# tskare/gpuaudiobench

Hardware: AMD Instinct MI355X
Metric: audio_buffers_per_sec (higher is better)
Workload: dtype f32

## Files before the change

### gpuaudiobench_amd/csrc/k_conv_accel.hip

```cpp
#include <hip/hip_runtime.h>
#include <hip/hip_ext.h>

#include <cmath>
#include <cstdlib>
#include <algorithm>
#include <chrono>
#include <memory>
#include <mutex>
#include <string>
#include <thread>
#include <type_traits>
#include <utility>
#include <vector>

#include "gab_common.hpp"
#include "gab_fft.hpp"
#include "gab_plan.hpp"
#include "k_conv_fdl.hpp"

namespace gab {
namespace fft {

void build_twiddles(float* t) {
    for (int m = 0; m < kTwiddleN; ++m) {
// ... 404 lines not shown
    load_spectra<kNB, 16>(cb, pmF + (size_t)q * kBinsB, tid);
    typename FB::Twiddles twb;
    FB::expand_twiddles(twb_base, twb);
    FB::run(zb, X, Y, twb, tid);
    cf zpb[16];
    partner_exchange<kNB, 16, true>(zb, zpb, X, tid);
    spectral_product<kNB, 16>(zb, zpb, cb, tid);
    FBi::template run<typename FB::Twiddles, 4>(zb, Y, X, twb, tid);
    cf* const c1 = cp + ((head + 1) & (kCarrySlots - 1)) * kB;
    cf* const c2 = cp + ((head + 2) & (kCarrySlots - 1)) * kB;
    c1[tid] = zb[12];
    c1[tid + kThreads] = zb[13];
    c2[tid] = zb[14];
    c2[tid + kThreads] = zb[15];
}

constexpr unsigned kRtSentinel = 0xffa5c3e1u;
__device__ __forceinline__ bool rt_pending(unsigned w) { return (w >> 24) == (kRtSentinel >> 24); }
constexpr size_t kRtUploadPiece = (size_t(4) << 20) - 256;
constexpr int kRtPollLimit = 1 << 21;
constexpr int kRtMaxGroups = 40;
constexpr size_t kBatchChunk = 256;
struct ConvRoundTrip {
    unsigned* stage;
    float* park;
    float* h_out;
    unsigned* counters;
    unsigned* done;
    const unsigned* landed;
    unsigned* error;
    unsigned epoch;
    int groups;
    unsigned bound[kRtMaxGroups + 1];
};

#ifdef GAB_ABLATE
__device__ unsigned long long g_rt_stamps[65 * 4];
#define GAB_RT_STAMP_MIN(g, i) do { if (threadIdx.x == 0) atomicMin(&g_rt_stamps[(g) * 4 + (i)], (unsigned long long)__builtin_amdgcn_s_memrealtime()); } while (0)
#define GAB_RT_STAMP_MAX(g, i) do { if (threadIdx.x == 0) atomicMax(&g_rt_stamps[(g) * 4 + (i)], (unsigned long long)__builtin_amdgcn_s_memrealtime()); } while (0)
#else
#define GAB_RT_STAMP_MIN(g, i) do {} while (0)
#define GAB_RT_STAMP_MAX(g, i) do {} while (0)
#endif

__device__ __forceinline__ unsigned rt_peek(const unsigned* p) {
    return __hip_atomic_load(p, __ATOMIC_RELAXED, __HIP_MEMORY_SCOPE_SYSTEM);
}
constexpr unsigned kRtErrWait = 1u, kRtErrTorn = 2u;

__global__ __launch_bounds__(kThreads) void conv_round_trip_check_kernel(unsigned* __restrict__ stage, const float* __restrict__ hist,
                                                                        unsigned* __restrict__ verdict, int slot) {
    const int tid = threadIdx.x, q = blockIdx.x;
    const cf* const hp = reinterpret_cast<const cf*>(hist) + ((size_t)q * kSlots + slot) * kB;
    unsigned* const row = stage + (size_t)(2 * q) * kB;
    const cf c0 = hp[tid], c1 = hp[tid + kThreads];
    const unsigned v0 = rt_peek(row + tid), v1 = rt_peek(row + tid + kThreads), v2 = rt_peek(row + kB + tid), v3 = rt_peek(row + kB + tid + kThreads);
    const bool torn = v0 != __float_as_uint(c0.x) || v2 != __float_as_uint(c0.y) || v1 != __float_as_uint(c1.x) || v3 != __float_as_uint(c1.y);
    if (torn) __hip_atomic_fetch_or(verdict, kRtErrTorn, __ATOMIC_RELAXED, __HIP_MEMORY_SCOPE_SYSTEM);
    __hip_atomic_store(row + tid, kRtSentinel, __ATOMIC_RELAXED, __HIP_MEMORY_SCOPE_SYSTEM);
    __hip_atomic_store(row + tid + kThreads, kRtSentinel, __ATOMIC_RELAXED, __HIP_MEMORY_SCOPE_SYSTEM);
    __hip_atomic_store(row + kB + tid, kRtSentinel, __ATOMIC_RELAXED, __HIP_MEMORY_SCOPE_SYSTEM);
    __hip_atomic_store(row + kB + tid + kThreads, kRtSentinel, __ATOMIC_RELAXED, __HIP_MEMORY_SCOPE_SYSTEM);
}

__global__ __launch_bounds__(kThreads, 2) void conv_round_trip_kernel(
    ConvRoundTrip rt, float* __restrict__ hist, const float4* __restrict__ pmA, const float4* __restrict__ pmB,
    const cf* __restrict__ tw, int T, int head) {
    __shared__ cf lds[2 * kLdsHalf];
    __shared__ int s_word;
    cf* const lds0 = lds;
    cf* const lds1 = lds + kLdsHalf;
    const int tid = threadIdx.x;
    const int q = blockIdx.x;
    const int ta = 2 * q;
    int g = 0;
    while (q >= (int)rt.bound[g + 1]) ++g;
    GAB_RT_STAMP_MIN(g, 0);
    cf* const hp = reinterpret_cast<cf*>(hist) + (size_t)q * kSlots * kB;
    using FA = fft::BlockFFT<kNA, 4, false>;
    using FAi = fft::BlockFFT<kNA, 4, true>;
    using FB = fft::BlockFFT<kNB, 16, false>;
    using FBi = fft::BlockFFT<kNB, 16, true>;

    cf zb[16];
    typename FB::Bases twb_base;
    FB::load_twiddles(twb_base, tw, tid);
#pragma unroll
    for (int r = 0; r < 16; ++r) zb[r] = hp[((head + (r >> 1)) & (kSlots - 1)) * kB + (r & 1) * kThreads + tid];
    const cf prev0 = zb[14], prev1 = zb[15];
    {
        float4 cb[16];
        load_spectra<kNB, 16>(cb, pmB + (size_t)q * kBinsB, tid);
        __builtin_amdgcn_sched_barrier(0);
        typename FB::Twiddles twb;
        FB::expand_twiddles(twb_base, twb);
        FB::run(zb, lds1, lds0, twb, tid);
        cf zpb[16];
        partner_exchange<kNB, 16, true>(zb, zpb, lds1, tid);
        spectral_product<kNB, 16>(zb, zpb, cb, tid);
        FBi::template run<typename FB::Twiddles, 2>(zb, lds0, lds1, twb, tid);
    }
    const cf far0 = zb[14], far1 = zb[15];

    float4 ca[4];
    load_spectra<kNA, 4>(ca, pmA + (size_t)q * kBinsA, tid);
    typename FA::Twiddles twa;
    {
        typename FA::Bases twa_base;
        FA::load_twiddles(twa_base, tw, tid);
        FA::expand_twiddles(twa_base, twa);
    }

    const unsigned* const row = rt.stage + (size_t)ta * kB;
    if (tid == 0) {
        int tries = 0, bad = 0;
        while (rt_pending(rt_peek(row + 2 * kB - 1))) {
            if ((++tries & 63) == 0 && rt_peek(rt.landed) == rt.epoch) break;
            if (tries > kRtPollLimit) { bad = 1; break; }
            __builtin_amdgcn_s_sleep(30);
        }
        s_word = bad;
    }
    __syncthreads();
    bool gave_up = s_word != 0;
    unsigned w[4];
    {
        int tries = 0;
        for (;;) {
            w[0] = rt_peek(row + tid);
            w[1] = rt_peek(row + tid + kThreads);
            w[2] = rt_peek(row + kB + tid);
            w[3] = rt_peek(row + kB + tid + kThreads);
            if (gave_up || !(rt_pending(w[0]) || rt_pending(w[1]) || rt_pending(w[2]) || rt_pending(w[3]))) break;
            if ((++tries & 15) == 0 && __hip_atomic_load(rt.landed, __ATOMIC_ACQUIRE, __HIP_MEMORY_SCOPE_SYSTEM) == rt.epoch) {
                w[0] = rt_peek(row + tid);
                w[1] = rt_peek(row + tid + kThreads);
                w[2] = rt_peek(row + kB + tid);
                w[3] = rt_peek(row + kB + tid + kThreads);
                break;
            }
            if (tries > kRtPollLimit) { gave_up = true; break; }
            __builtin_amdgcn_s_sleep(10);
        }
    }
    GAB_RT_STAMP_MAX(g, 1);
    if (gave_up) __hip_atomic_store(rt.error, kRtErrWait, __ATOMIC_RELAXED, __HIP_MEMORY_SCOPE_SYSTEM);

    cf za[4];
    za[0] = prev0;
    za[1] = prev1;
    za[2] = mk(__uint_as_float(w[0]), __uint_as_float(w[2]));
    za[3] = mk(__uint_as_float(w[1]), __uint_as_float(w[3]));
    hp[head * kB + tid] = za[2];
    hp[head * kB + kThreads + tid] = za[3];
    __syncthreads();
    FA::run(za, lds0, lds1, twa, tid);
    {
        cf zpa[4];
        partner_exchange<kNA, 4, true>(za, zpa, lds0, tid);
        spectral_product<kNA, 4>(za, zpa, ca, tid);
    }
    FAi::run(za, lds1, lds0, twa, tid);
    float ya0 = 0.f, yb0 = 0.f, ya1 = 0.f, yb1 = 0.f;
    ya0 += za[2].x; yb0 += za[2].y; ya1 += za[3].x; yb1 += za[3].y;
    ya0 += far0.x; yb0 += far0.y; ya1 += far1.x; yb1 += far1.y;

    {
        unsigned long long* const p0 = reinterpret_cast<unsigned long long*>(rt.park + (size_t)T * tid + ta);
        unsigned long long* const p1 = reinterpret_cast<unsigned long long*>(rt.park + (size_t)T * (tid + kThreads) + ta);
        const unsigned long long v0 = ((unsigned long long)__float_as_uint(yb0) << 32) | __float_as_uint(ya0);
        const unsigned long long v1 = ((unsigned long long)__float_as_uint(yb1) << 32) | __float_as_uint(ya1);
        __hip_atomic_store(p0, v0, __ATOMIC_RELAXED, __HIP_MEMORY_SCOPE_AGENT);
        __hip_atomic_store(p1, v1, __ATOMIC_RELAXED, __HIP_MEMORY_SCOPE_AGENT);
    }
    asm volatile("s_waitcnt vmcnt(0)" ::: "memory");
    __syncthreads();
    GAB_RT_STAMP_MAX(g, 2);
    const int first = rt.bound[g];
    const int members = (int)rt.bound[g + 1] - first;
    unsigned* const gw = rt.counters + 32 * g;
    if (tid == 0) {
        const unsigned old = __hip_atomic_fetch_add(&gw[0], 1u, __ATOMIC_RELAXED, __HIP_MEMORY_SCOPE_AGENT);
        int role = 1;
        if (old + 1u == rt.epoch * (unsigned)members) {
            role = 2;
            __hip_atomic_store(&gw[1], 0u, __ATOMIC_RELAXED, __HIP_MEMORY_SCOPE_AGENT);
            asm volatile("s_waitcnt vmcnt(0)" ::: "memory");
            __hip_atomic_store(&gw[2], rt.epoch, __ATOMIC_RELAXED, __HIP_MEMORY_SCOPE_AGENT);
        } else {
            int tries = 0;
            while (__hip_atomic_load(&gw[2], __ATOMIC_RELAXED, __HIP_MEMORY_SCOPE_AGENT) != rt.epoch) {
                if (++tries > (1 << 10)) { role = 0; break; }
                __builtin_amdgcn_s_sleep(3);
            }
        }
        s_word = role;
    }
    __syncthreads();
    const int role = s_word;
    if (role == 0) return;
    const int row_f4 = members / 2;
    const auto srd = __builtin_amdgcn_make_buffer_rsrc(rt.park, 0, (int)((size_t)T * kB * 4), 0x00020000);
    const int col0 = 2 * first;
    unsigned drained = 0;
    for (;;) {
        __syncthreads();
        if (tid == 0) s_word = (int)__hip_atomic_fetch_add(&gw[1], 1u, __ATOMIC_RELAXED, __HIP_MEMORY_SCOPE_AGENT);
        __syncthreads();
        const int share = s_word;
        if (share >= members) break;
        const int i = share * kThreads + tid;
        const int sidx = i / row_f4, c = i - sidx * row_f4;
        const auto raw = __builtin_amdgcn_raw_buffer_load_b128(srd, 4u * (unsigned)(T * sidx + col0 + 4 * c), 0, 16);
        typedef float f4v __attribute__((ext_vector_type(4)));
        const f4v val = {__uint_as_float(raw[0]), __uint_as_float(raw[1]), __uint_as_float(raw[2]), __uint_as_float(raw[3])};
        float* const dst = rt.h_out + (size_t)T * sidx + col0 + 4 * c;
        asm volatile("global_store_dwordx4 %0, %1, off sc0 sc1" ::"v"(dst), "v"(val) : "memory");
        ++drained;
        if (role != 2) break;
    }
    asm volatile("s_waitcnt vmcnt(0)" ::: "memory");
    __syncthreads();
    GAB_RT_STAMP_MAX(g, 3);
    if (tid == 0 && drained) {
        const unsigned old = __hip_atomic_fetch_add(&rt.counters[32 * rt.groups], drained, __ATOMIC_RELAXED, __HIP_MEMORY_SCOPE_AGENT);
        if (old + drained == rt.epoch * (unsigned)gridDim.x) {
            __hip_atomic_store(rt.done, rt.epoch, __ATOMIC_RELAXED, __HIP_MEMORY_SCOPE_SYSTEM);
            GAB_RT_STAMP_MAX(64, 0);
        }
    }
}

__global__ __launch_bounds__(kThreads, 2) void conv_batch_kernel(
    const float* __restrict__ in, float* __restrict__ out, float* __restrict__ hist,
    const float4* __restrict__ pmA, const float4* __restrict__ pmB,
    const cf* __restrict__ tw, int T, int head, int n_buffers) {
    __shared__ cf lds[2 * kLdsHalf];
    const size_t step = (size_t)T * kB;
    for (int nb = 0; nb < n_buffers; ++nb)
        conv_one_buffer<true, true, true>(in + nb * step, out + nb * step, hist, pmA, pmB, tw, T,
                                             (head + nb) & (kSlots - 1), lds);
}

constexpr int kBatchBarriers = 6;

struct ConvEngine {
    const unsigned* doorbell;
    unsigned* relay;
    unsigned* progress;
    unsigned* completed;
    unsigned* error;
    int ring;
    int poll_every_period;
    unsigned* started;
    unsigned* resident;
    unsigned long long idle_ticks;
};
constexpr double kEngineIdleSeconds = 4.0;

typedef unsigned u4 __attribute__((ext_vector_type(4)));

constexpr int kB12Threads = 768;
constexpr int kB12SpecCf = 4 * kBinsA * 2;
constexpr int kB12Tw1Cf = 16 * 15;
constexpr int kB12Lds = 6 * kWaveImg + 2 * kLdsHalf + kB12SpecCf + kB12Tw1Cf;

template <int N, int R, int R0, int R1, class PM>
__device__ __forceinline__ void load_spectra_part(float4 (&c)[R1 - R0], PM pm, int tid) {
    constexpr int NT = N / R;
#pragma unroll
    for (int r = R0; r < R1; ++r) {
        const int k = tid + r * NT;
        if (r < R / 2) c[r - R0] = pm[k];
        else if (r > R / 2) c[r - R0] = pm[N - k];
        else c[r - R0] = pm[tid == 0 ? k : N - k];
    }
}
template <int N, int R, int R0, int R1>
__device__ __forceinline__ void spectral_product_part(cf (&z)[R], const cf (&zraw)[R1 - R0], const float4 (&c)[R1 - R0], int tid) {
#pragma unroll
    for (int r = R0; r < R1; ++r) {
        cf P = mk(c[r - R0].x, c[r - R0].y), M = mk(c[r - R0].z, c[r - R0].w);
        if (r > R / 2 || (r == R / 2 && tid != 0)) z[r] = fft::cfma_cjcj(zraw[r - R0], M, fft::cmulc(z[r], P));
        else z[r] = fft::cfma_cj(zraw[r - R0], M, fft::cmul(z[r], P));
    }
}
template <int N, int R, int R0, int R1>
__device__ __forceinline__ void spectral_product_partner_part(cf (&wp)[R1 - R0], const cf (&z)[R], const cf (&zp)[R1 - R0], const float4 (&c)[R1 - R0]) {
    static_assert(R1 <= R / 2, "the partners of the low bins");
#pragma unroll
    for (int r = R0; r < R1; ++r) {
        cf P = mk(c[r - R0].x, c[r - R0].y), M = mk(c[r - R0].z, c[r - R0].w);
        wp[r - R0] = fft::cfma_cjcj(z[r], M, fft::cmulc(zp[r - R0], P));
    }
}
template <int R0, int R1>
__device__ __forceinline__ void near_product_half(cf (&v)[16], const cf* fimg, const float4* sp_lds, int lane) {
    cf zp[R1 - R0];
    float4 ch[R1 - R0];
#pragma unroll
    for (int r = R0; r < R1; ++r) zp[r - R0] = fimg[PadA16::at((kNA - (lane + 64 * r)) & (kNA - 1))];
    load_spectra_part<kNA, 16, R0, R1>(ch, sp_lds, lane);
    spectral_product_part<kNA, 16, R0, R1>(v, zp, ch, lane);
}

#ifdef GAB_ABLATE
__device__ unsigned long long g_split_stamps[2 * 8 * 8192];
#define GAB_B12BAR(period, i)                                                                                         \
    do {                                                                                                              \
        if ((sp.debug & 64) && ((period) == 32 || (period) == 33) && lane == 0)                                       \
            g_split_stamps[(((size_t)blockIdx.x * 12 + w) * 2 + ((period) - 32)) * 6 + (i)] = __builtin_amdgcn_s_memrealtime(); \
        __syncthreads();                                                                                              \
    } while (0)
#else
#define GAB_B12BAR(period, i) __syncthreads()
#endif
__device__ __forceinline__ void conv_split_batch12_resident(
    const float* __restrict__ in, float* __restrict__ out, float* __restrict__ hist,
    const float4* __restrict__ pmA, const ConvSplit& sp, const cf* __restrict__ tw, int T, int head0, int n_buffers,
    cf* __restrict__ lds) {
    cf* const far_img = lds + 6 * kWaveImg;
    float4* const spec = reinterpret_cast<float4*>(far_img + 2 * kLdsHalf);
    cf* const tw1 = reinterpret_cast<cf*>(spec + 4 * kBinsA);
    const int tid = threadIdx.x;
    const int d = xcd_contiguous(blockIdx.x, gridDim.x);
    const size_t step = (size_t)T * kB;
    {
        const float4* const gA = pmA + (size_t)(2 * d) * kBinsA;
        const float4* const gA2 = sp.pmA2 + (size_t)(2 * d) * kBinsA;
        for (int i = tid; i < 2 * kBinsA; i += kB12Threads) { spec[i] = gA[i]; spec[2 * kBinsA + i] = gA2[i]; }
        if (tid < 16) {
            cf pw[15];
            fft::powers_of<16>(tw[tid * (fft::kTwiddleN / 256)], pw);
#pragma unroll
            for (int r = 0; r < 15; ++r) tw1[tid * 15 + r] = pw[r];
        }
    }
    __syncthreads();
    const int lane = tid & 63;
    const int w = __builtin_amdgcn_readfirstlane(tid >> 6);
    const unsigned rb = (unsigned)lane + ((unsigned)lane >> 4);
    auto in_slot = [&](int slot) -> const float* { return in + (size_t)slot * step; };
    auto idle_period = [&]() { for (int i = 0; i < kBatchBarriers; ++i) __syncthreads(); };

    if (w >= 4) {
        const int g = __builtin_amdgcn_readfirstlane((w - 4) >> 2);
        const int ft = (tid - kThreads) & (kThreads - 1);
        cf* const img = far_img + g * kLdsHalf;
        const int q = 2 * d + g;
        const cf* const hp = reinterpret_cast<const cf*>(hist) + (size_t)q * kSlots * kB;
        cf* const cg = sp.carry + (size_t)q * kCarrySlots * kB;
        const size_t ca = (size_t)(2 * q) * kB, cb_ = ca + kB;
        const float4* const pf = sp.pmF + (size_t)q * kBinsB;
        using B16 = fft::Butterfly<16, false>;
        using B16i = fft::Butterfly<16, true>;
        cf tw2[15];
        fft::powers_of<16>(tw[ft], tw2);
        auto opaque_t = [&]() -> unsigned { unsigned v = (unsigned)ft; asm volatile("" : "+v"(v)); return v; };
        auto w0_of = [](unsigned t) -> unsigned { return t * 17u; };
        auto rd_of = [](unsigned t) -> unsigned { return t + (t >> 4); };
        auto w1_of = [](unsigned t) -> unsigned { const unsigned b1 = (t >> 4) * 256u + (t & 15u); return b1 + (b1 >> 4); };
        auto tw1row_of = [&](unsigned t) -> const cf* { return tw1 + (t & 15u) * 15u; };
        auto load_window = [&](auto part_tag, int nb, cf (&z)[16]) {
            constexpr int PART = decltype(part_tag)::value;
            const int head = (head0 + nb) & (kSlots - 1);
            int fo = ft;
            asm volatile("" : "+v"(fo));
            if constexpr (PART == 0) {
                const float* const cur = in_slot(nb);
                z[14] = mk(cur[ca + fo], cur[cb_ + fo]);
                z[15] = mk(cur[ca + fo + kThreads], cur[cb_ + fo + kThreads]);
            }
            constexpr int BL0 = PART == 0 ? 4 : 0, BL1 = PART == 0 ? 7 : 4;
            if (nb >= kSlots - 1) {
#pragma unroll
                for (int bl = BL0; bl < BL1; ++bl) {
                    const float* const src = in_slot(nb - (7 - bl));
                    z[2 * bl] = mk(src[ca + fo], src[cb_ + fo]);
                    z[2 * bl + 1] = mk(src[ca + fo + kThreads], src[cb_ + fo + kThreads]);
                }
            } else {
#pragma unroll
                for (int bl = BL0; bl < BL1; ++bl) {
                    if (nb - 7 + bl >= 0) {
                        const float* const src = in_slot(nb - (7 - bl));
                        z[2 * bl] = mk(src[ca + fo], src[cb_ + fo]);
                        z[2 * bl + 1] = mk(src[ca + fo + kThreads], src[cb_ + fo + kThreads]);
                    } else {
                        const int s = ((head + 1 + bl) & (kSlots - 1)) * kB;
                        z[2 * bl] = hp[s + fo];
                        z[2 * bl + 1] = hp[s + kThreads + fo];
                    }
                }
            }
        };
        cf z[16], zn[16];
#ifdef GAB_ABLATE
        const bool own_bins = (sp.debug & 128) != 0;
#else
        constexpr bool own_bins = false;
#endif
        auto first_half = [&](int nb) {
#pragma unroll
            for (int r = 0; r < 16; ++r) z[r] = zn[r];
            B16::run(z);
            {
                const unsigned w0 = w0_of(opaque_t());
#pragma unroll
                for (int r = 0; r < 16; ++r) img[w0 + r] = z[B16::out_slot(r)];
            }
            GAB_B12BAR(nb, 0);
            {
                const unsigned t = opaque_t(), rd = rd_of(t);
                const cf* const tw1row = tw1row_of(t);
#pragma unroll
                for (int r = 0; r < 16; ++r) z[r] = img[rd + 272 * r];
#pragma unroll
                for (int r = 1; r < 16; ++r) z[r] = fft::cmul(z[r], tw1row[r - 1]);
            }
            B16::run(z);
            GAB_B12BAR(nb, 1);
            {
                const unsigned w1 = w1_of(opaque_t());
#pragma unroll
                for (int r = 0; r < 16; ++r) img[w1 + 17 * r] = z[B16::out_slot(r)];
            }
            __builtin_amdgcn_sched_barrier(0);
            float4 clo[8], cny = make_float4(0.0f, 0.0f, 0.0f, 0.0f);
            {
                int fo = ft;
                asm volatile("" : "+v"(fo));
                load_spectra_part<kNB, 16, 0, 8>(clo, pf, fo);
                if (fo == 0) cny = pf[kNB / 2];
            }
            __builtin_amdgcn_sched_barrier(0);
            GAB_B12BAR(nb, 2);
            {
                const unsigned rd = rd_of(opaque_t());
#pragma unroll
                for (int r = 0; r < 16; ++r) z[r] = img[rd + 272 * r];
            }
#pragma unroll
            for (int r = 1; r < 16; ++r) z[r] = fft::cmul(z[r], tw2[r - 1]);
            B16::run(z);
            GAB_B12BAR(nb, 3);
#ifdef GAB_ABLATE
            if (own_bins) {
                {
                    const unsigned t = opaque_t();
#pragma unroll
                    for (int r = 0; r < 16; ++r) img[t + 256u * r] = z[B16::out_slot(r)];
                }
                GAB_B12BAR(nb, 4);
                cf o[16];
#pragma unroll
                for (int r = 0; r < 16; ++r) o[r] = z[B16::out_slot(r)];
#pragma unroll
                for (int r = 0; r < 16; ++r) z[r] = o[r];
                const unsigned t = opaque_t();
                const cf* const pb = img + (kNB - 256 * 15) - t;
                cf zp[8];
                zp[0] = img[(kNB - t) & (kNB - 1)];
#pragma unroll
                for (int r = 1; r < 8; ++r) zp[r] = pb[256 * (15 - r)];
                spectral_product_part<kNB, 16, 0, 8>(z, zp, clo, ft);
                load_spectra_part<kNB, 16, 8, 16>(clo, pf, ft);
#pragma unroll
                for (int r = 0; r < 8; ++r) zp[r] = pb[256 * (7 - r)];
                spectral_product_part<kNB, 16, 8, 16>(z, zp, clo, ft);
                GAB_B12BAR(nb, 5);
                return;
            }
#endif
            {
                const unsigned t = opaque_t();
#pragma unroll
                for (int r = 8; r < 16; ++r) img[t + 256u * (r - 8)] = z[B16::out_slot(r)];
            }
            GAB_B12BAR(nb, 4);
            {
                cf o[16];
#pragma unroll
                for (int r = 0; r < 16; ++r) o[r] = z[B16::out_slot(r)];
#pragma unroll
                for (int r = 0; r < 16; ++r) z[r] = o[r];
                const unsigned t = opaque_t();
                const cf* const pb = img + (kNB / 2 - 256 * 7) - t;
                cf zp[8], wp[8];
                zp[0] = img[(kNB / 2 - t) & (kNB / 2 - 1)];
                if (t == 0) zp[0] = z[0];
#pragma unroll
                for (int r = 1; r < 8; ++r) zp[r] = pb[256 * (7 - r)];
                spectral_product_partner_part<kNB, 16, 0, 8>(wp, z, zp, clo);
                spectral_product_part<kNB, 16, 0, 8>(z, zp, clo, ft);
                if (t == 0) {
                    const cf P = mk(cny.x, cny.y), M = mk(cny.z, cny.w);
                    wp[0] = fft::cfma_cj(z[8], M, fft::cmul(z[8], P));
                }
                cf* const qb = img + kNB / 2 + (kNB / 2 - 256 * 7) - t;
                img[kNB / 2 + ((kNB / 2 - t) & (kNB / 2 - 1))] = wp[0];
#pragma unroll
                for (int r = 1; r < 8; ++r) qb[256 * (7 - r)] = wp[r];
            }
            GAB_B12BAR(nb, 5);
        };
        auto second_half = [&](int period, int nb_done, int nb_next) {
            if (nb_next >= 0) {
                load_window(std::integral_constant<int, 0>{}, nb_next, zn);
            } else {
#pragma unroll
                for (int r = 0; r < 16; ++r) zn[r] = mk(0.0f, 0.0f);
            }
            __builtin_amdgcn_sched_barrier(0);
            if (nb_done >= 0) {
                if (!own_bins) {
                    const unsigned t = opaque_t();
#pragma unroll
                    for (int r = 8; r < 16; ++r) z[r] = img[kNB / 2 + t + 256u * (r - 8)];
                }
                B16i::run(z);
            }
            GAB_B12BAR(period, 0);
            if (nb_done >= 0) {
                const unsigned w0 = w0_of(opaque_t());
#pragma unroll
                for (int r = 0; r < 16; ++r) img[w0 + r] = z[B16i::out_slot(r)];
            }
            GAB_B12BAR(period, 1);
            if (nb_done >= 0) {
                const unsigned t = opaque_t(), rd = rd_of(t);
                const cf* const tw1row = tw1row_of(t);
#pragma unroll
                for (int r = 0; r < 16; ++r) z[r] = img[rd + 272 * r];
#pragma unroll
                for (int r = 1; r < 16; ++r) z[r] = fft::cmulc(z[r], tw1row[r - 1]);
                B16i::run(z);
            }
            GAB_B12BAR(period, 2);
            if (nb_done >= 0) {
                const unsigned w1 = w1_of(opaque_t());
#pragma unroll
                for (int r = 0; r < 16; ++r) img[w1 + 17 * r] = z[B16i::out_slot(r)];
            }
            __builtin_amdgcn_sched_barrier(0);
            if (nb_next >= 0) load_window(std::integral_constant<int, 1>{}, nb_next, zn);
            __builtin_amdgcn_sched_barrier(0);
            GAB_B12BAR(period, 3);
            if (nb_done >= 0) {
                const unsigned rd = rd_of(opaque_t());
#pragma unroll
                for (int r = 0; r < 16; ++r) z[r] = img[rd + 272 * r];
#pragma unroll
                for (int r = 1; r < 16; ++r) z[r] = fft::cmulc(z[r], tw2[r - 1]);
                cf x12, x13, x14, x15;
                B16i::run_last4(z, x12, x13, x14, x15);
                const int head = (head0 + nb_done) & (kSlots - 1);
                cf* const c1 = cg + ((head + 1) & (kCarrySlots - 1)) * kB;
                cf* const c2 = cg + ((head + 2) & (kCarrySlots - 1)) * kB;
                c1[ft] = x12;
                c1[ft + kThreads] = x13;
                c2[ft] = x14;
                c2[ft + kThreads] = x15;
            }
            GAB_B12BAR(period, 4);
            if (nb_done >= 0) asm volatile("s_waitcnt vmcnt(0)" ::: "memory");
            GAB_B12BAR(period, 5);
        };
        const int first = (g - head0) & 1;
        int nb = 0;
        if (first == 0 && n_buffers > 0) {
            load_window(std::integral_constant<int, 0>{}, 0, zn);
            load_window(std::integral_constant<int, 1>{}, 0, zn);
        }
        __syncthreads();
        if (first == 1) {
            second_half(0, -1, 1 < n_buffers ? 1 : -1);
            nb = 1;
        }
        for (;;) {
            if (nb > n_buffers) break;
            if (nb < n_buffers) first_half(nb); else idle_period();
            ++nb;
            if (nb > n_buffers) break;
            second_half(nb, nb - 1 < n_buffers ? nb - 1 : -1, nb + 1 < n_buffers ? nb + 1 : -1);
            ++nb;
        }
    } else if (w < 2) {
        const int q = 2 * d + w;
        cf* const hp = reinterpret_cast<cf*>(hist) + (size_t)q * kSlots * kB;
        cf* const img = lds + w * kWaveImg;
        cf* const hand = lds + (2 + w) * kWaveImg;
        const float4* const sa = spec + w * kBinsA;
        const float4* const sa2 = spec + (2 + w) * kBinsA;
        using WF = fft::WaveFFT1024<false>;
        WF::Lean t;
        WF::load_twiddles(t, tw, lane);
        const size_t xoff = (size_t)(2 * q) * kB;
        cf z[16], prev[8], nxt[8];
        {
            const int s1 = ((head0 + kSlots - 1) & (kSlots - 1)) * kB, s2 = ((head0 + kSlots - 2) & (kSlots - 1)) * kB;
#pragma unroll
            for (int j = 0; j < 8; ++j) z[j] = hp[s2 + lane + 64 * j];
#pragma unroll
            for (int j = 0; j < 8; ++j) prev[j] = hp[s1 + lane + 64 * j];
            if (n_buffers > 0) {
                const float* const x0 = in_slot(0) + xoff;
#pragma unroll
                for (int j = 0; j < 8; ++j) nxt[j] = mk(x0[lane + 64 * j], x0[kB + lane + 64 * j]);
            }
#pragma unroll
            for (int j = 0; j < 8; ++j) z[8 + j] = prev[j];
            WF::run(z, img, t, lane, WF::NoHook());
#pragma unroll
            for (int r = 0; r < 16; ++r) img[rb + 68 * r] = z[r];
            __syncthreads();
        }
        for (int nb = 0; nb < n_buffers; ++nb) {
            const int head = (head0 + nb) & (kSlots - 1);
            cf share[16];
#pragma unroll
            for (int r = 0; r < 8; ++r) share[r] = img[rb + 68 * r];
            near_product_half<0, 8>(share, img, sa2, lane);
            GAB_B12BAR(nb, 0);
            __builtin_amdgcn_sched_barrier(0);
#pragma unroll
            for (int j = 0; j < 8; ++j) { z[j] = prev[j]; z[8 + j] = nxt[j]; }
            if (nb + kSlots >= n_buffers) {
#pragma unroll
                for (int j = 0; j < 8; ++j) hp[head * kB + lane + 64 * j] = nxt[j];
            }
#pragma unroll
            for (int j = 0; j < 8; ++j) prev[j] = nxt[j];
            if (nb + 1 < n_buffers) {
                int lo = lane;
                asm volatile("" : "+v"(lo));
                const float* const xa = in_slot(nb + 1) + xoff + lo;
#pragma unroll
                for (int j = 0; j < 8; ++j) nxt[j] = mk(xa[64 * j], xa[kB + 64 * j]);
            }
            WF::run(z, img, t, lane, [&](int i) { GAB_B12BAR(nb, 1 + i); });
#pragma unroll
            for (int r = 0; r < 16; ++r) img[rb + 68 * r] = z[r];
            GAB_B12BAR(nb, 3);
            near_product_half<0, 8>(z, img, sa, lane);
            GAB_B12BAR(nb, 4);
#pragma unroll
            for (int r = 0; r < 8; ++r) hand[rb + 68 * r] = fft::cadd(z[r], share[r]);
            GAB_B12BAR(nb, 5);
        }
        idle_period();
    } else {
        const int pr = w - 2;
        cf* const hand = lds + (2 + pr) * kWaveImg;
        const cf* const fimg = lds + pr * kWaveImg;
        const float4* const sa = spec + pr * kBinsA;
        const float4* const sa2 = spec + (2 + pr) * kBinsA;
        cf* const img = lds + (4 + pr) * kWaveImg;
        const cf* const other = lds + (4 + (1 - pr)) * kWaveImg;
        const cf* const cg = sp.carry + (size_t)(2 * d + pr) * kCarrySlots * kB;
        using WFi = fft::WaveFFT1024<true>;
        WFi::Lean t;
        WFi::load_twiddles(t, tw, lane);
        cf ws[16], sum[8];
        auto product_half = [&](const float4* sp_lds) {
#pragma unroll
            for (int r = 8; r < 16; ++r) ws[r] = fimg[rb + 68 * r];
            near_product_half<8, 16>(ws, fimg, sp_lds, lane);
        };
        auto store_share = [&]() {
#pragma unroll
            for (int r = 8; r < 16; ++r) hand[rb + 68 * r] = ws[r];
        };
        auto sum_halves = [&]() {
#pragma unroll
            for (int j = 0; j < 8; ++j) sum[j] = fft::cadd(ws[8 + j], hand[rb + 68 * (8 + j)]);
        };
        __syncthreads();
        if (n_buffers > 0) {
            product_half(sa2);
            GAB_B12BAR(0, 0);
            store_share();
            GAB_B12BAR(0, 1);
            GAB_B12BAR(0, 2);
            GAB_B12BAR(0, 3);
            product_half(sa);
            GAB_B12BAR(0, 4);
            sum_halves();
            GAB_B12BAR(0, 5);
        } else {
            idle_period();
        }
        for (int nb = 1; nb <= n_buffers; ++nb) {
            const bool products = nb < n_buffers;
            const int b = nb - 1;
            const int head = (head0 + b) & (kSlots - 1);
            float* const outb = out + (size_t)b * step;
            cf z[16], y[8], park[8];
#pragma unroll
            for (int r = 0; r < 8; ++r) z[r] = hand[rb + 68 * r];
#pragma unroll
            for (int j = 0; j < 8; ++j) z[8 + j] = sum[j];
            {
                int lo = lane;
                asm volatile("" : "+v"(lo));
                const unsigned long long* const cy = reinterpret_cast<const unsigned long long*>(cg + (head & (kCarrySlots - 1)) * kB + lo);
#pragma unroll
                for (int j = 0; j < 8; ++j) {
                    const unsigned long long v = __hip_atomic_load(cy + 64 * j, __ATOMIC_RELAXED, __HIP_MEMORY_SCOPE_AGENT);
                    park[j] = mk(__uint_as_float((unsigned)v), __uint_as_float((unsigned)(v >> 32)));
                }
            }
            __builtin_amdgcn_sched_barrier(0);
            if (products) product_half(sa2);
            GAB_B12BAR(nb, 0);
            if (products) store_share();
            __builtin_amdgcn_sched_barrier(0);
            WFi::run(z, img, t, lane, [&](int i) { GAB_B12BAR(nb, 1 + i); });
#pragma unroll
            for (int j = 0; j < 8; ++j) y[j] = fft::cadd(z[8 + j], park[j]);
            GAB_B12BAR(nb, 3);
            if (pr == 0) {
#pragma unroll
                for (int j = 0; j < 4; ++j) img[lane + 64 * j] = y[4 + j];
            } else {
#pragma unroll
                for (int j = 0; j < 4; ++j) img[lane + 64 * j] = y[j];
            }
            __builtin_amdgcn_sched_barrier(0);
            if (products) product_half(sa);
            GAB_B12BAR(nb, 4);
            {
                float* const o0 = outb + 4 * (size_t)d;
                if (pr == 0) {
#pragma unroll
                    for (int j = 0; j < 4; ++j) {
                        const cf theirs = other[lane + 64 * j];
                        *reinterpret_cast<float4*>(o0 + (size_t)T * (lane + 64 * j)) = make_float4(y[j].x, y[j].y, theirs.x, theirs.y);
                    }
                } else {
#pragma unroll
                    for (int j = 0; j < 4; ++j) {
                        const cf theirs = other[lane + 64 * j];
                        *reinterpret_cast<float4*>(o0 + (size_t)T * (lane + 64 * (4 + j))) = make_float4(theirs.x, theirs.y, y[4 + j].x, y[4 + j].y);
                    }
                }
            }
            if (products) sum_halves();
            GAB_B12BAR(nb, 5);
        }
    }
}

__global__ __launch_bounds__(kB12Threads) void conv_split_batch12_kernel(
    const float* __restrict__ in, float* __restrict__ out, float* __restrict__ hist,
    const float4* __restrict__ pmA, ConvSplit sp, const cf* __restrict__ tw, int T, int head0, int n_buffers) {
    __shared__ __attribute__((aligned(16))) cf lds[kB12Lds];
    conv_split_batch12_resident(in, out, hist, pmA, sp, tw, T, head0, n_buffers, lds);
}

#ifdef GAB_ABLATE
#define GAB_E12BAR(i)                                                                                                 \
    do {                                                                                                              \
        if ((sp.debug & 64) && (nb == 4000 || nb == 4001) && lane == 0)                                               \
            g_split_stamps[(((size_t)blockIdx.x * 12 + w) * 2 + (nb - 4000)) * 6 + (i)] = __builtin_amdgcn_s_memrealtime(); \
        __syncthreads();                                                                                              \
    } while (0)
#else
#define GAB_E12BAR(i) __syncthreads()
#endif
__device__ __forceinline__ void conv_split_engine12_resident(
    const float* __restrict__ in, float* __restrict__ out, float* __restrict__ hist,
    const float4* __restrict__ pmA, const ConvSplit& sp, const cf* __restrict__ tw, int T, int head0,
    const ConvEngine& eng, cf* __restrict__ lds, unsigned* __restrict__ s_door) {
    constexpr bool ENGINE = true;
    constexpr int n_buffers = 0;
    (void)ENGINE; (void)n_buffers;
    cf* const far_img = lds + 6 * kWaveImg;
    float4* const spec = reinterpret_cast<float4*>(far_img + 2 * kLdsHalf);
    cf* const tw1 = reinterpret_cast<cf*>(spec + 4 * kBinsA);
    const int tid = threadIdx.x;
    const int d = xcd_contiguous(blockIdx.x, gridDim.x);
    const size_t step = (size_t)T * kB;
    {
        const float4* const gA = pmA + (size_t)(2 * d) * kBinsA;
        const float4* const gA2 = sp.pmA2 + (size_t)(2 * d) * kBinsA;
        for (int i = tid; i < 2 * kBinsA; i += kB12Threads) { spec[i] = gA[i]; spec[2 * kBinsA + i] = gA2[i]; }
        if (tid < 16) {
            cf pw[15];
            fft::powers_of<16>(tw[tid * (fft::kTwiddleN / 256)], pw);
#pragma unroll
            for (int r = 0; r < 15; ++r) tw1[tid * 15 + r] = pw[r];
        }
    }
    constexpr int kPoller = 2 * 64;
    auto read_door = [&]() -> unsigned {
        if (blockIdx.x == 0) {
            const unsigned v = __hip_atomic_load(eng.doorbell, __ATOMIC_RELAXED, __HIP_MEMORY_SCOPE_SYSTEM);
            __hip_atomic_store(eng.relay, v, __ATOMIC_RELAXED, __HIP_MEMORY_SCOPE_AGENT);
            return v;
        }
        return __hip_atomic_load(eng.relay, __ATOMIC_RELAXED, __HIP_MEMORY_SCOPE_AGENT);
    };
    if (tid == 0) {
        s_door[2] = 0;
        const unsigned before = __hip_atomic_fetch_add(eng.started, 1u, __ATOMIC_RELAXED, __HIP_MEMORY_SCOPE_AGENT);
        if (before == 0) __hip_atomic_store(&eng.resident[0], 1u, __ATOMIC_RELAXED, __HIP_MEMORY_SCOPE_SYSTEM);
        if (before + 1 == gridDim.x) __hip_atomic_store(&eng.resident[1], gridDim.x, __ATOMIC_RELAXED, __HIP_MEMORY_SCOPE_SYSTEM);
    }
    __syncthreads();
    const int lane = tid & 63;
    const int w = __builtin_amdgcn_readfirstlane(tid >> 6);
    const unsigned rb = (unsigned)lane + ((unsigned)lane >> 4);
    const bool aggregator = blockIdx.x == (gridDim.x > 1 ? 1u : 0u);
    unsigned reported = 0;
    auto aggregate_request = [&](u4& a, u4& b) {
        const auto srd = __builtin_amdgcn_make_buffer_rsrc(eng.progress, 0, (int)(8u * gridDim.x), 0x00020000);
        a = __builtin_amdgcn_raw_buffer_load_b128(srd, 32u * (unsigned)lane, 0, 16);
        b = __builtin_amdgcn_raw_buffer_load_b128(srd, 32u * (unsigned)lane + 16u, 0, 16);
    };
    auto aggregate_report = [&](const u4& a, const u4& b) {
        const unsigned words = 2u * gridDim.x;
        auto pick = [&](unsigned v, unsigned idx) { return idx < words ? v : 0xffffffffu; };
        unsigned m = min(min(min(pick(a[0], 8u * lane), pick(a[1], 8u * lane + 1)), min(pick(a[2], 8u * lane + 2), pick(a[3], 8u * lane + 3))),
                         min(min(pick(b[0], 8u * lane + 4), pick(b[1], 8u * lane + 5)), min(pick(b[2], 8u * lane + 6), pick(b[3], 8u * lane + 7))));
// ... 1823 lines not shown
```

Baseline: 213,300.

## Pair mirror bins in-register via lane-half swaps instead of LDS round trip

Remaps which frequency bins each far-path thread owns so that a bin and its conjugate partner live in the two halves of the same wavefront. The partner values are then exchanged with cross-lane half swaps rather than being written to and read back from LDS. This removes LDS stores and loads in the spectral product stage and the second-half reload. In exchange it adds cross-lane permute traffic and special-case selects for lanes 0 and 32 of the first wave, and it changes the thread-to-bin mapping that other stages rely on.

```diff
diff --git a/gpuaudiobench_amd/csrc/k_conv_accel.hip b/gpuaudiobench_amd/csrc/k_conv_accel.hip
--- a/gpuaudiobench_amd/csrc/k_conv_accel.hip
+++ b/gpuaudiobench_amd/csrc/k_conv_accel.hip
@@ -730,6 +730,12 @@
     for (int r = R0; r < R1; ++r) zp[r - R0] = fimg[PadA16::at((kNA - (lane + 64 * r)) & (kNA - 1))];
     load_spectra_part<kNA, 16, R0, R1>(ch, sp_lds, lane);
     spectral_product_part<kNA, 16, R0, R1>(v, zp, ch, lane);
+}
+
+__device__ __forceinline__ void trade_lane_halves(cf& a, cf& b) {
+    using WF = fft::WaveFFT1024<false>;
+    WF::swap_lane_halves<32>(a, b);
+    WF::swap_lane_halves<32>(b, a);
 }
 
 #ifdef GAB_ABLATE
@@ -773,7 +779,8 @@
 
     if (w >= 4) {
         const int g = __builtin_amdgcn_readfirstlane((w - 4) >> 2);
-        const int ft = (tid - kThreads) & (kThreads - 1);
+        const int fw = (w - 4) & 3;
+        const int ft = lane < 32 ? 32 * fw + lane : ((fw | (lane & 31)) == 0 ? kThreads / 2 : kThreads - 32 * fw - (lane & 31));
         cf* const img = far_img + g * kLdsHalf;
         const int q = 2 * d + g;
         const cf* const hp = reinterpret_cast<const cf*>(hist) + (size_t)q * kSlots * kB;
@@ -825,8 +832,6 @@
         cf z[16], zn[16];
 #ifdef GAB_ABLATE
         const bool own_bins = (sp.debug & 128) != 0;
-#else
-        constexpr bool own_bins = false;
 #endif
         auto first_half = [&](int nb) {
 #pragma unroll
@@ -900,35 +905,44 @@
                 return;
             }
 #endif
-            {
-                const unsigned t = opaque_t();
-#pragma unroll
-                for (int r = 8; r < 16; ++r) img[t + 256u * (r - 8)] = z[B16::out_slot(r)];
-            }
-            GAB_B12BAR(nb, 4);
+            cf zp[8], wp[8];
             {
                 cf o[16];
 #pragma unroll
                 for (int r = 0; r < 16; ++r) o[r] = z[B16::out_slot(r)];
 #pragma unroll
                 for (int r = 0; r < 16; ++r) z[r] = o[r];
-                const unsigned t = opaque_t();
-                const cf* const pb = img + (kNB / 2 - 256 * 7) - t;
-                cf zp[8], wp[8];
-                zp[0] = img[(kNB / 2 - t) & (kNB / 2 - 1)];
-                if (t == 0) zp[0] = z[0];
-#pragma unroll
-                for (int r = 1; r < 8; ++r) zp[r] = pb[256 * (7 - r)];
-                spectral_product_partner_part<kNB, 16, 0, 8>(wp, z, zp, clo);
-                spectral_product_part<kNB, 16, 0, 8>(z, zp, clo, ft);
-                if (t == 0) {
-                    const cf P = mk(cny.x, cny.y), M = mk(cny.z, cny.w);
-                    wp[0] = fft::cfma_cj(z[8], M, fft::cmul(z[8], P));
+#pragma unroll
+                for (int i = 0; i < 4; ++i) {
+                    zp[i] = z[8 + i];
+                    zp[7 - i] = z[15 - i];
+                    trade_lane_halves(zp[i], zp[7 - i]);
                 }
-                cf* const qb = img + kNB / 2 + (kNB / 2 - 256 * 7) - t;
-                img[kNB / 2 + ((kNB / 2 - t) & (kNB / 2 - 1))] = wp[0];
-#pragma unroll
-                for (int r = 1; r < 8; ++r) qb[256 * (7 - r)] = wp[r];
+                if (fw == 0) {
+                    const bool t0 = lane == 0, t128 = lane == 32;
+                    zp[0] = t0 ? z[0] : t128 ? z[15] : zp[0];
+#pragma unroll
+                    for (int r = 1; r < 8; ++r) zp[r] = t0 ? z[16 - r] : t128 ? z[15 - r] : zp[r];
+                }
+            }
+            GAB_B12BAR(nb, 4);
+            spectral_product_partner_part<kNB, 16, 0, 8>(wp, z, zp, clo);
+            spectral_product_part<kNB, 16, 0, 8>(z, zp, clo, ft);
+            if (ft == 0) {
+                const cf P = mk(cny.x, cny.y), M = mk(cny.z, cny.w);
+                wp[0] = fft::cfma_cj(z[8], M, fft::cmul(z[8], P));
+            }
+#pragma unroll
+            for (int i = 0; i < 4; ++i) {
+                z[8 + i] = wp[i];
+                z[15 - i] = wp[7 - i];
+                trade_lane_halves(z[8 + i], z[15 - i]);
+            }
+            if (fw == 0) {
+                const bool t0 = lane == 0, t128 = lane == 32;
+                z[8] = t0 ? wp[0] : t128 ? wp[7] : z[8];
+#pragma unroll
+                for (int r = 9; r < 16; ++r) z[r] = t0 ? wp[16 - r] : t128 ? wp[15 - r] : z[r];
             }
             GAB_B12BAR(nb, 5);
         };
@@ -940,14 +954,7 @@
                 for (int r = 0; r < 16; ++r) zn[r] = mk(0.0f, 0.0f);
             }
             __builtin_amdgcn_sched_barrier(0);
-            if (nb_done >= 0) {
-                if (!own_bins) {
-                    const unsigned t = opaque_t();
-#pragma unroll
-                    for (int r = 8; r < 16; ++r) z[r] = img[kNB / 2 + t + 256u * (r - 8)];
-                }
-                B16i::run(z);
-            }
+            if (nb_done >= 0) B16i::run(z);
             GAB_B12BAR(period, 0);
             if (nb_done >= 0) {
                 const unsigned w0 = w0_of(opaque_t());
```

After: 215,700, median of 6. +1.2%, better.
